# pityka/lamp

Hardware: AMD Instinct MI355X
Metric: training-step samples/sec (higher is better)
Workload: dtype bf16; 1 GPU; example-cifar100 Cnn.resnet(100) training step (fwd+backprop+AdamW), synthetic CIFAR batch; per_gpu_batch=2048, global_batch=2048, parallelism=single, optimizer=AdamW lr 1e-3 wd 0 beta2 0.95 mixedPrecision

## Files before the change

### lamp_amd/csrc/core/switches.h

```cpp
#pragma once
#include <cstdint>

namespace lamp {

constexpr int64_t SW_NO_CLAMP = INT64_MIN;

#define LAMP_SWITCHES_ONCE(X)                                                                                                             \
                                                        \
  X(conv_sibling, "LAMP_CONV_SIBLING", BOOL, 1, 0, "a residual block's 3x3 and its sibling 1x1 of the same input as one forward launch") \
  X(fuse_bn_pair, "LAMP_FUSE_BN_PAIR", BOOL, 1, 0, "relu(bn(right) + bn(left)) at a block's end as one op (0: the chain)")                \
  X(fuse_pool_logsoftmax, "LAMP_FUSE_POOL_LOGSOFTMAX", BOOL, 1, 0, "average pool -> flatten -> log-softmax tail as one node")             \
  X(fuse_block_tail, "LAMP_FUSE_BLOCK_TAIL", BOOL, 1, 0, "the last residual block and the pooled log-softmax tail as one node")          \
  X(fuse_bn_conv, "LAMP_FUSE_BN_CONV", BOOL, 1, 0, "batch norm -> relu -> convolution: the convolution applies the norm while staging")  \
  X(fuse_loss_accumulate, "LAMP_FUSE_LOSS_ACCUMULATE", BOOL, 1, 0, "acc += n * loss inside the NLL loss kernel")                          \
  X(fuse_loss_backward, "LAMP_FUSE_LOSS_BACKWARD", BOOL, 1, 0, "the NLL loss backward goes straight to the pooled log-softmax node's input in one launch")                      \
  X(fuse_loss_tail, "LAMP_FUSE_LOSS_TAIL", BOOL, 1, 0, "the loss launch also writes the pooled log-softmax's input gradient per plane")  \
  X(conv_dgrad_accumulate, "LAMP_CONV_DGRAD_ACCUMULATE", BOOL, 1, 0, "a convolution's input gradient adds into the existing one in its epilogue") \
  X(conv_dgrad_pair, "LAMP_CONV_DGRAD_PAIR", BOOL, 1, 0, "input gradients of a block's 3x3 and sibling 1x1 from one launch")             \
  X(conv_wgrad_pair, "LAMP_CONV_WGRAD_PAIR", BOOL, 1, 0, "weight gradients of a block's 3x3 and sibling 1x1 from one launch")            \
  X(linear_bias_fused, "LAMP_LINEAR_BIAS_FUSED", BOOL, 1, 0, "a linear layer's bias in the GEMM epilogue (0: mm then add)")               \
  X(mult_add_fused, "LAMP_MULT_ADD_FUSED", BOOL, 1, 0, "x * scale + residual in one pass (0: mult then add)")                             \
  X(attention_as_written_for_cuda, "LAMP_ATTENTION_AS_WRITTEN_FOR_CUDA", BOOL, 0, 0, "multi-head attention as the reference's op chain instead of the fused kernels") \
  X(recurrent_fused, "LAMP_RECURRENT_FUSED", BOOL, 1, 0, "RNN / GRU / LSTM as one node per sequence with fused cell kernels (0: the fold over time steps)") \
  X(fuse_qkv, "LAMP_FUSE_QKV", BOOL, 1, 0, "self-attention's three projections as one product (0: three)")                                \
  X(host_stream_side, "LAMP_HOST_STREAM_SIDE", BOOL, 0, 0, "batch streams gather on a side stream instead of the consumer's")             \
                                                                           \
  X(pinned_cache_mb, "LAMP_PINNED_CACHE_MB", INT, 2048, 0, "upper bound of the cache of freed pinned host buffers, MiB")                  \
  X(pinned_gather_wgs, "LAMP_PINNED_GATHER_WGS", INT, 48, 1, "workgroups of a gather that reads pinned host memory")                      \
                                                                                                    \
  X(flash_attention, "LAMP_FLASH_ATTENTION", BOOL, 1, 0, "the flash attention kernels, forward and backward")                             \
  X(small_attention, "LAMP_SMALL_ATTENTION", BOOL, 1, 0, "the short-sequence attention kernels")                                          \
  X(knn_fused, "LAMP_KNN_FUSED", BOOL, 1, 0, "the fused distance + top-k nearest-neighbour kernel")                                       \
  X(knn_split, "LAMP_KNN_SPLIT", INT, -1, SW_NO_CLAMP, "f16-plane k-NN filter: 0 off, 1 where it pays, 2 forced; negative: the mode set through the API") \
  X(knn_split_planes, "LAMP_KNN_SPLIT_PLANES", INT, 0, SW_NO_CLAMP, "f16 planes per coordinate of that filter: 3, anything else 2")      \
  X(umap_pairs2, "LAMP_UMAP_PAIRS2", BOOL, 1, 0, "the UMAP loss's two-dimensional pair kernel")                                            \
                                                                                                             \
  X(gemm_shape_tags, "LAMP_GEMM_SHAPE_TAGS", BOOL, 0, 0, "profiling aid: one kernel-timer class per GEMM shape and layout")               \
  X(gemm_splitk, "LAMP_GEMM_SPLITK", BOOL, 1, 0, "split-K for products with few output tiles (bf16 and f32 / f64)")                       \
  X(gemm_tail_split, "LAMP_GEMM_TAIL_SPLIT", BOOL, 1, 0, "an almost empty last round of 256 x 256 tiles becomes a second, split-K product") \
  X(gemm_fp_split_wgs, "LAMP_GEMM_FP_SPLIT_WGS", INT, 512, 1, "workgroups an f32 / f64 split-K product aims at")                          \
                                                                                              \
  X(bn_fused_bwd, "LAMP_BN_FUSED_BWD", BOOL, 1, 0, "one-pass batch-norm backward (workgroups exchange their sums) where no mode is set through the API") \
  X(bn_fused_fp, "LAMP_BN_FUSED_FP", BOOL, 1, 0, "... its f32 / f64 form")                                                               \
  X(bn_fused_np_mask, "LAMP_BN_FUSED_NP_MASK", INT, 24, SW_NO_CLAMP, "bit mask of packets per thread (1 .. 16) at which the one-pass form runs") \
  X(bn_fused_per_cu, "LAMP_BN_FUSED_PER_CU", INT, 1, 1, "workgroups per CU the one-pass form aims at first")                              \
  X(bn_fused_small_bytes, "LAMP_BN_FUSED_SMALL_BYTES", INT, (4 << 20) + 1, SW_NO_CLAMP, "bf16 activations below this many bytes take the one-pass form whatever the mask") \
                          \
  X(conv_small2, "LAMP_CONV_SMALL2", BOOL, 1, 0, "the small-map direct convolution kernels (second generation)")                          \
  X(conv_small2_wgrad, "LAMP_CONV_SMALL2_WGRAD", BOOL, 1, 0, "... their weight gradient")                                                 \
  X(igemm_f32, "LAMP_IGEMM_F32", BOOL, 1, 0, "implicit-GEMM convolution for f32")                                                          \
  X(igemm_f64, "LAMP_IGEMM_F64", BOOL, 1, 0, "implicit-GEMM convolution for f64")                                                          \
  X(conv_bn_stats, "LAMP_CONV_BN_STATS", BOOL, 1, 0, "forward convolutions hand per-image batch-norm statistics of their output on")     \
  X(ncv_bn_stats, "LAMP_NCV_BN_STATS", BOOL, 1, 0, "... the narrow kernels' alone (needs LAMP_CONV_BN_STATS on as well)")                 \
  X(ncv_dgrad_parity, "LAMP_NCV_DGRAD_PARITY", BOOL, 1, 0, "narrow stride-2 pair input gradient: super-tiles by row parity (0: the plain form)") \
  X(ncv_pitch, "LAMP_NCV_PITCH", BOOL, 1, 0, "narrow kernels widen the LDS row pitch to a bank-conflict-free one")                        \
  X(ncv_two_shift, "LAMP_NCV_TWO_SHIFT", BOOL, 1, 0, "narrow kernels: two output phases per MFMA where the columns allow it")             \
  X(ncv_per_cu, "LAMP_NCV_PER_CU", INT, 4, 1, "narrow kernels: most workgroups per CU")                                                   \
  X(pack_cache, "LAMP_PACK_CACHE", BOOL, 1, 0, "packed filter images are cached per parameter and storage version (all four packing backends: core/pack_cache.h)") \
  X(pack_after_step, "LAMP_PACK_AFTER_STEP", BOOL, 1, 0, "the optimiser repacks every cached filter image of all four backends in place (0: lazily at first use)") \
                                                    \
  X(ig_small_d, "LAMP_IG_SMALL_D", BOOL, 1, 0, "the eight-image kernel for at most 64 output channels too")                               \
  X(ig_w8, "LAMP_IG_W8", BOOL, 1, 0, "two-image 128-row kernel: eight waves per image pair at one workgroup per CU or fewer (0: four)")  \
  X(ig_one_image, "LAMP_IG_ONE_IMAGE", BOOL, 1, 0, "... one image per workgroup at one image per CU or fewer (0: pairs)")                 \
                                                                                                 \
  X(wgrad_group, "LAMP_WGRAD_GROUP", BOOL, 1, 0, "two layers' eight-wave weight gradients parked and launched as one (0: every layer at once)") \
  X(wgrad_min_ips, "LAMP_WGRAD_MIN_IPS", INT, 0, 2, "fewest images per weight-gradient workgroup; unset (0): 2 up to 512 images, 8 above") \
  X(wg8h_dma, "LAMP_WG8H_DMA", BOOL, 1, 0, "eight-wave weight-gradient kernel: dY tiles by LDS-DMA (0: through registers, the bitwise reference of the DMA's hand-counted waits)") \
  X(defer_wgrad_reduce, "LAMP_DEFER_WGRAD_REDUCE", BOOL, 1, 0, "weight-gradient partial sums are reduced in batches, deferred until someone reads them")

#define LAMP_SWITCHES_PER_CALL(X)                                                                                                         \
  X(ig_variant, "LAMP_IG_VARIANT", LETTER, 0, 0, "bf16 implicit GEMM kernel form: b two-image 128-row, d eight-image at any batch; unset or any other letter: by geometry") \
  X(ig_ktail, "LAMP_IG_KTAIL", BOOL, 1, 0, "a 3x3's 1 .. 8 channels beyond the last whole K chunk from their own packed image (0: the padded chunk)") \
  X(knn_split_dbg, "LAMP_KNN_SPLIT_DBG", INT, 0, SW_NO_CLAMP, "3: the k-NN filter's kernel counts visits, candidates and selection cycles per wave and prints them")

using SwType_BOOL = bool;
using SwType_INT = int64_t;
using SwType_LETTER = char;
#define LAMP_SWITCH_MEMBER(member, name, kind, dflt, lo, doc) SwType_##kind member;
struct Switches { LAMP_SWITCHES_ONCE(LAMP_SWITCH_MEMBER) };
struct SwitchesNow { LAMP_SWITCHES_PER_CALL(LAMP_SWITCH_MEMBER) };
#undef LAMP_SWITCH_MEMBER

const Switches& sw();
SwitchesNow sw_now();

}
```

### lamp_amd/csrc/kernels/conv_igemm.hip

```cpp
#include "device_utils.h"
#include "conv_geom.h"
#include "conv_backends.h"
#include "../core/pack_cache.h"
#include "wgrad_reduce.h"
#include <thread>
#include "conv_narrow_pack.h"
#include "../core/switches.h"

namespace lamp {

typedef short s8v __attribute__((ext_vector_type(8)));
typedef __bf16 bf8v __attribute__((ext_vector_type(8)));
typedef float f4v __attribute__((ext_vector_type(4)));

constexpr int IG_M = 128;
constexpr int IG_WTILE = 128 * 64 * 2;

__device__ __forceinline__ int ig_kc_off(int row, int chunk) { return row * 128 + ((chunk ^ (row & 7)) << 4); }

__device__ __forceinline__ void ig_stage_load_rows(uint4 (&r)[4], const bf16_t* __restrict__ base, int64_t ld, int64_t k0, int64_t rows,
                                                   int64_t K, int tid) {
#pragma unroll
  for (int i = 0; i < 4; i++) {
    const int c = tid + i * 256;
// ... 487 lines not shown
    const int qrow = (q == 1 || q == 2) ? 1 : 0, qw = (q >= 2) ? 4 : 0;
#pragma unroll
    for (int i = 0; i < 2; i++) {
      const int co = wr * 32 + i * 16 + (lane & 15);
      const float b = (bias && co < CO) ? (float)bias[co] : 0.f;
      float vals[16];
#pragma unroll
      for (int j = 0; j < 4; j++) {
        const bf16_t o0(acc[i][j][0] + b), o1(acc[i][j][1] + b), o2(acc[i][j][2] + b), o3(acc[i][j][3] + b);
        if (co < CO) {
          uint2 pk;
          pk.x = (unsigned)o0.bits | ((unsigned)o1.bits << 16);
          pk.y = (unsigned)o2.bits | ((unsigned)o3.bits << 16);
          if (addend) {
            const uint2 av = *reinterpret_cast<const uint2*>(addend + (int64_t)n * CO * 64 + co * 64 + (2 * j + qrow) * 8 + qw);
            pk.x = add_bf16x2(pk.x, av.x); pk.y = add_bf16x2(pk.y, av.y);
          }
          *reinterpret_cast<uint2*>(yp + co * 64 + (2 * j + qrow) * 8 + qw) = pk;
        }
        vals[4 * j + 0] = __uint_as_float((unsigned)o0.bits << 16); vals[4 * j + 1] = __uint_as_float((unsigned)o1.bits << 16);
        vals[4 * j + 2] = __uint_as_float((unsigned)o2.bits << 16); vals[4 * j + 3] = __uint_as_float((unsigned)o3.bits << 16);
      }
      if (stats) {
        float wn, wm, w2;
        ig_stats_wave(vals, wn, wm, w2);
        if (q == 0 && co < CO) { float* sp = stats + ((int64_t)co * N + n) * 3;  sp[0] = wn; sp[1] = wm; sp[2] = w2; }
      }
    }
  }
}

__device__ __forceinline__ uint4 ig_bn_relu_x8(uint4 v, float mu, float scale, float bb) {
  unsigned* w = &v.x;
#pragma unroll
  for (int q = 0; q < 4; q++) {
    const float x0 = __uint_as_float(w[q] << 16), x1 = __uint_as_float(w[q] & 0xffff0000u);
    bf16_t o0(__builtin_fmaf(x0 - mu, scale, bb)), o1(__builtin_fmaf(x1 - mu, scale, bb));
    if ((float)o0 < 0.f) o0 = bf16_t(0.f);
    if ((float)o1 < 0.f) o1 = bf16_t(0.f);
    w[q] = (unsigned)o0.bits | ((unsigned)o1.bits << 16);
  }
  return v;
}

#ifdef IG8D_STAMP
__device__ unsigned long long ig8d_stamps[8 * 512];
__device__ unsigned long long ig8d_rt_stamps[8 * 512];
#define IG_STAMP(k) do { if (threadIdx.x == 0 && blockIdx.x < 512) { ig8d_stamps[blockIdx.x * 8 + (k)] = __builtin_amdgcn_s_memtime(); \
                                                                     ig8d_rt_stamps[blockIdx.x * 8 + (k)] = __builtin_amdgcn_s_memrealtime(); } } while (0)
#else
#define IG_STAMP(k) do { } while (0)
#endif
__device__ __forceinline__ int ig8d_swz(int h, int w) { return ((h & 1) << 1) | ((w >> 2) & 1); }

__device__ __forceinline__ void ig8d_tile_stats(const uint2 (&pk)[4], float& mean, float& m2) {
  typedef float f2v __attribute__((ext_vector_type(2)));
  const float sh = __uint_as_float(pk[0].x << 16);
  const f2v sh2 = {sh, sh};
  f2v s1 = {0.f, 0.f}, s2 = {0.f, 0.f};
#pragma unroll
  for (int j = 0; j < 4; j++) {
    const f2v va = {__uint_as_float(pk[j].x << 16), __uint_as_float(pk[j].x & 0xffff0000u)};
    const f2v vb = {__uint_as_float(pk[j].y << 16), __uint_as_float(pk[j].y & 0xffff0000u)};
    const f2v da = va - sh2, db = vb - sh2;
    s1 += da; s2 = __builtin_elementwise_fma(da, da, s2);
    s1 += db; s2 = __builtin_elementwise_fma(db, db, s2);
  }
  const float t1 = s1[0] + s1[1], t2 = s2[0] + s2[1];
  mean = sh + t1 * (1.f / 16.f); m2 = t2 - t1 * t1 * (1.f / 16.f);
  {
    float ma = mean, mb = mean, qa = m2, qb = m2;
    asm("s_nop 1\n\tv_permlane16_swap_b32 %0, %1" : "+v"(ma), "+v"(mb));
    asm("s_nop 1\n\tv_permlane16_swap_b32 %0, %1" : "+v"(qa), "+v"(qb));
    const float d = mb - ma; mean = ma + d * 0.5f; m2 = qa + qb + d * d * 8.f;
  }
  {
    float ma = mean, mb = mean, qa = m2, qb = m2;
    asm("s_nop 1\n\tv_permlane32_swap_b32 %0, %1" : "+v"(ma), "+v"(mb));
    asm("s_nop 1\n\tv_permlane32_swap_b32 %0, %1" : "+v"(qa), "+v"(qb));
    const float d = mb - ma; mean = ma + d * 0.5f; m2 = qa + qb + d * d * 16.f;
  }
}

template <int KS, int NCT, int SIBM>
__global__ __launch_bounds__(512) void ig_conv8d_kernel(const bf16_t* __restrict__ x, const bf16_t* __restrict__ wp, const bf16_t* __restrict__ bias,
                                                        bf16_t* y, int N, int CI, int KP, int CO, float* __restrict__ stats, int stats_per_wg,
                                                        const bf16_t* addend, const float4* __restrict__ affine, const IgSibling sib) {
  constexpr bool SIB = SIBM == 1, DG2 = SIBM == 2;
  static_assert(SIBM == 0 || KS == 3, "the sibling product is the centre tap of a 3x3 staging");
  extern __shared__ __attribute__((aligned(16))) char smem[];
  constexpr int RS = KS * KS;
  constexpr int PAD = (KS - 1) / 2;
  constexpr int NI = 8, NT = 512;
  constexpr int WT = 128 * 32 * 2, NSLOT = 3;
  constexpr int RB = 64;
  constexpr int XIMG = 64 * RB;
  constexpr int XBUF = NI * XIMG;
  char* Wl = smem;
  char* Xl = smem + NSLOT * WT;
  const int tid = threadIdx.x, lane = tid & 63;
  const int wid = __builtin_amdgcn_readfirstlane(tid >> 6);
  const int grp = wid >> 2;
  const int n0 = blockIdx.x * NI;
  const int KC = (CI + 31) >> 5;
  const bool tailm = KS == 3 && !SIB && sib.wtail != nullptr;
  const int KCF = tailm ? KC - 1 : KC;
  const int T = RS * KCF + (tailm ? IG_TAIL_STAGES : 0);

  typedef __attribute__((address_space(3))) char lds_char_t;
  typedef const __attribute__((address_space(1))) char glb_char_t;
  const int d_row = wid * 16 + (lane >> 2);
  const unsigned d_src = (unsigned)(d_row * KP + (((lane & 3) ^ ((4 - ((d_row >> 2) & 3)) & 3)) << 3)) * 2u;
  const unsigned d_src4 = d_src + 64u * (unsigned)KP * 2u;
  constexpr int NPIECE = SIB ? 2 : 1;
  const bool dma_wave = SIB ? wid < 4 : wid < NCT;
  auto stage_dma_of = [&](const bf16_t* wimg, int kc1, int rs1, int slot) {
    const char* base = reinterpret_cast<const char*>(wimg + (int64_t)rs1 * IG_M * KP + kc1 * 32);
    if constexpr (SIB) {
      if (wid < 4) {
        __builtin_amdgcn_global_load_lds((glb_char_t*)(base + d_src), (lds_char_t*)(Wl + slot * WT + wid * 1024), 16, 0, 0);
        __builtin_amdgcn_global_load_lds((glb_char_t*)(base + d_src4), (lds_char_t*)(Wl + slot * WT + (wid + 4) * 1024), 16, 0, 0);
      }
    } else {
      if (wid < NCT)
        __builtin_amdgcn_global_load_lds((glb_char_t*)(base + d_src), (lds_char_t*)(Wl + slot * WT + wid * 1024), 16, 0, 0);
    }
  };
  const unsigned d_srct = (unsigned)(d_row * 32 + (((lane & 3) ^ ((4 - ((d_row >> 2) & 3)) & 3)) << 3)) * 2u;
  auto stage_dma = [&](int kc1, int rs1, int slot) {
    if (kc1 < KCF) { stage_dma_of(wp, kc1, rs1, slot); return; }
    if constexpr (!SIB) {
      const char* base = reinterpret_cast<const char*>(sib.wtail + ((kc1 - KCF) * RS + rs1) * (IG_M * 32));
      if (wid < NCT) __builtin_amdgcn_global_load_lds((glb_char_t*)(base + d_srct), (lds_char_t*)(Wl + slot * WT + wid * 1024), 16, 0, 0);
    }
  };
  constexpr bool WIDE = NCT == 1 && !SIB;
  const unsigned d_srcw = (unsigned)((lane >> 2) * KP + wid * 32 + (((lane & 3) ^ ((4 - ((lane >> 4) & 3)) & 3)) << 3)) * 2u;
  auto stage_dma_w = [&](const bf16_t* wimg, int rs1, int slot) {
    if (wid < KC)
      __builtin_amdgcn_global_load_lds((glb_char_t*)(reinterpret_cast<const char*>(wimg + (int64_t)rs1 * IG_M * KP) + d_srcw),
                                       (lds_char_t*)(Wl + slot * WT + wid * 1024), 16, 0, 0);
  };
  const bool taps4 = WIDE && !DG2 && KC == 1 && RS > 1;
  auto stage_dma_t = [&](int g, int slot) {
    const int tap = 4 * g + wid;
    if (wid < 4 && tap < RS)
      __builtin_amdgcn_global_load_lds((glb_char_t*)(reinterpret_cast<const char*>(wp + (int64_t)tap * IG_M * KP) + (d_srcw - (unsigned)(wid * 32) * 2u)),
                                       (lds_char_t*)(Wl + slot * WT + wid * 1024), 16, 0, 0);
  };
  IG_STAMP(0);
  if constexpr (WIDE) {
    if (taps4) { stage_dma_t(0, 0); stage_dma_t(1, 1); }
    else if (DG2) { stage_dma_w(sib.wp, 0, 0); stage_dma_w(wp, 0, 1); }
    else { stage_dma_w(wp, 0, 0); if (RS > 1) stage_dma_w(wp, 1, 1); }
  } else if (SIB || DG2) {
    stage_dma_of(sib.wp, 0, 0, 0);
    if (KC > 1) stage_dma_of(sib.wp, 1, 0, 1);
  } else {
    stage_dma(0, 0, 0);
    if (T > 1) stage_dma(1 / RS, 1 % RS, 1);
  }
  IG_STAMP(1);
  unsigned bpair[SIB ? (NCT + 1) / 2 : 1];
  if constexpr (SIB) {
#pragma unroll
    for (int k = 0; k < (NCT + 1) / 2; k++) {
      const int c0 = 2 * k * 16 + (lane & 15), c1 = c0 + 16;
      const unsigned b0 = (sib.bias && c0 < CO) ? sib.bias[c0].bits : 0u, b1 = (sib.bias && 2 * k + 1 < NCT && c1 < CO) ? sib.bias[c1].bits : 0u;
      bpair[k] = b0 | (b1 << 16);
    }
  }
  auto load_images = [&](const bf16_t* __restrict__ x) {
    for (int e = tid; e < NI * 8 * 4 * KC; e += NT) {
      const int cg = e & 3, h = (e >> 2) & 7, img = (e >> 5) & 7, ch = e >> 8;
      const int n = n0 + img;
      uint4 rw[8];
#pragma unroll
      for (int k = 0; k < 8; k++) {
        const int c = ch * 32 + cg * 8 + k;
        rw[k] = make_uint4(0, 0, 0, 0);
        if (c < CI && n < N) {
          const uint4* src = reinterpret_cast<const uint4*>(x + ((int64_t)n * CI + c) * 64 + h * 8);
          rw[k] = stats ? nt_load16(src) : *src;
        }
      }
      if (affine) {
#pragma unroll
        for (int k = 0; k < 8; k++) {
          const int c = ch * 32 + cg * 8 + k;
          if (c < CI && n < N) { const float4 a = affine[c]; rw[k] = ig_bn_relu_x8(rw[k], a.x, a.y, a.z); }
        }
      }
      char* xi = Xl + ch * XBUF + img * XIMG;
#pragma unroll
      for (int p = 0; p < 8; p++) {
        unsigned int d[4];
#pragma unroll
        for (int j = 0; j < 4; j++) {
          const unsigned int lo = (&rw[2 * j].x)[p >> 1], hi = (&rw[2 * j + 1].x)[p >> 1];
          d[j] = (p & 1) ? ((lo >> 16) | (hi & 0xffff0000u)) : ((lo & 0xffffu) | (hi << 16));
        }
        *reinterpret_cast<uint4*>(xi + (h * 8 + p) * RB + ((cg ^ ig8d_swz(h, p)) << 4)) = make_uint4(d[0], d[1], d[2], d[3]);
      }
    }
  };
  load_images(DG2 ? sib.x2 : x);
  f4v acc[NCT][4];
#pragma unroll
  for (int i = 0; i < NCT; i++)
#pragma unroll
    for (int j = 0; j < 4; j++) acc[i][j] = f4v{0.f, 0.f, 0.f, 0.f};

  int rowsel, wpix;
  px_of_col(lane & 15, rowsel, wpix);
  const int p0 = wid * XIMG + ((rowsel - PAD) * 8 + (wpix - PAD)) * RB;
  int va[2][KS];
#pragma unroll
  for (int par = 0; par < 2; par++)
#pragma unroll
    for (int s = 0; s < KS; s++)
      va[par][s] = p0 + (((lane >> 4) ^ ig8d_swz(rowsel + par - PAD, wpix + s - PAD)) << 4);
  const bool col_lo = wpix == 0, col_hi = wpix == 7, row_lo = rowsel == 0, row_hi = rowsel == 1;
  const int a_off = (lane & 15) * 64 + ((((lane >> 4) ^ ((4 - ((lane >> 2) & 3)) & 3)) & 3) << 4);

  asm volatile("s_waitcnt vmcnt(0) lgkmcnt(0)" ::: "memory");
  __builtin_amdgcn_s_barrier();
  if constexpr (SIB) {
#pragma unroll
    for (int k = 0; k < (NCT + 1) / 2; k++) asm volatile("" : "+v"(bpair[k]));
  }
  IG_STAMP(2);

  bf8v fa[NCT], fb[4];
  const bf8v zero8 = __builtin_bit_cast(bf8v, s8v{0, 0, 0, 0, 0, 0, 0, 0});
  if constexpr (WIDE) {
    bf8v fw[4], fx[4][4];
    auto read_stage = [&](int slot, int r, int s) {
      const char* wl = Wl + slot * WT + a_off;
#pragma unroll
      for (int kc = 0; kc < 4; kc++)
        if (kc < KC) {
          fw[kc] = __builtin_bit_cast(bf8v, *reinterpret_cast<const s8v*>(wl + kc * 1024));
          const char* xb = Xl + kc * XBUF + va[r & 1][s];
#pragma unroll
          for (int j = 0; j < 4; j++) fx[kc][j] = __builtin_bit_cast(bf8v, *reinterpret_cast<const s8v*>(xb + ((r * 8 + s) + 16 * j) * RB));
        }
    };
    auto zero_outside = [&](int r, int s) {
      if (KS != 3) return;
      const bool colout = (s == 0 && col_lo) || (s == 2 && col_hi);
#pragma unroll
      for (int kc = 0; kc < 4; kc++)
        if (kc < KC) {
#pragma unroll
          for (int j = 0; j < 4; j++) {
            const bool out = colout || (r == 0 && j == 0 && row_lo) || (r == 2 && j == 3 && row_hi);
            if (s != 1 || (r == 0 && j == 0) || (r == 2 && j == 3)) fx[kc][j] = out ? zero8 : fx[kc][j];
          }
        }
    };
    auto multiply = [&] {
      __builtin_amdgcn_s_setprio(1);
#pragma unroll
      for (int kc = 0; kc < 4; kc++)
        if (kc < KC) {
#pragma unroll
          for (int j = 0; j < 4; j++) acc[0][j] = __builtin_amdgcn_mfma_f32_16x16x32_bf16(fx[kc][j], fw[kc], acc[0][j], 0, 0, 0);
        }
      __builtin_amdgcn_s_setprio(0);
    };
    int slot = 0;
    if (taps4) {
      constexpr int NG = (RS + 3) / 4;
      if (grp == 1) __builtin_amdgcn_s_barrier();
#pragma unroll
      for (int g = 0; g < NG; g++) {
        const int slot1 = slot == 2 ? 0 : slot + 1, slot2 = slot1 == 2 ? 0 : slot1 + 1;
        if (g + 2 < NG) stage_dma_t(g + 2, slot2);
        const char* wl = Wl + slot * WT + a_off;
#pragma unroll
        for (int p = 0; p < 4; p++) {
          const int tap = 4 * g + p;
          if (tap < RS) {
            const int r = tap / KS, s_ = tap - r * KS;
            fw[p] = __builtin_bit_cast(bf8v, *reinterpret_cast<const s8v*>(wl + p * 1024));
            const char* xb = Xl + va[r & 1][s_];
#pragma unroll
            for (int j = 0; j < 4; j++) fx[p][j] = __builtin_bit_cast(bf8v, *reinterpret_cast<const s8v*>(xb + ((r * 8 + s_) + 16 * j) * RB));
          }
        }
        if (g + 2 < NG) asm volatile("s_waitcnt vmcnt(1) lgkmcnt(0)" ::: "memory");
        else asm volatile("s_waitcnt vmcnt(0) lgkmcnt(0)" ::: "memory");
        if (KS == 3) {
#pragma unroll
          for (int p = 0; p < 4; p++) {
            const int tap = 4 * g + p;
            if (tap < RS) {
              const int r = tap / KS, s_ = tap - r * KS;
              const bool colout = (s_ == 0 && col_lo) || (s_ == 2 && col_hi);
#pragma unroll
              for (int j = 0; j < 4; j++) {
                const bool out = colout || (r == 0 && j == 0 && row_lo) || (r == 2 && j == 3 && row_hi);
                if (s_ != 1 || (r == 0 && j == 0) || (r == 2 && j == 3)) fx[p][j] = out ? zero8 : fx[p][j];
              }
            }
          }
        }
        __builtin_amdgcn_s_barrier();
        __builtin_amdgcn_s_setprio(1);
#pragma unroll
        for (int p = 0; p < 4; p++)
          if (4 * g + p < RS) {
// ... 741 lines not shown
      if (co < CO2 && ci < CI) __builtin_nontemporal_store(acc2[i], reinterpret_cast<f4v*>(&out2[co * CIP + ci]));
    }
  }
#pragma unroll
  for (int t = 0; t < RS; t++) {
    float* out = partial + (int64_t)(split * RS + t) * IG_M * CIP;
#pragma unroll
    for (int i = 0; i < 2; i++) {
      const int ci = ci0 + i * 16 + (lane >> 4) * 4;
      if (co < CO && ci < CI) __builtin_nontemporal_store(acc[t][i], reinterpret_cast<f4v*>(&out[co * CIP + ci]));
    }
  }
}

static bool ig_qualifies(const ConvGeom& g, int dtype) {
  if (dtype != kBF16) return false;
  if (g.groups != 1 || g.transposed) return false;
  if (g.H != 8 || g.W != 8 || g.Ho != 8 || g.Wo != 8) return false;
  if (g.sh != 1 || g.sw != 1 || g.dh != 1 || g.dw != 1) return false;
  if (!((g.kh == 3 && g.kw == 3 && g.ph == 1 && g.pw == 1) || (g.kh == 1 && g.kw == 1 && g.ph == 0 && g.pw == 0))) return false;
  if (g.Cin > 128 || g.Cout > 128 || g.Cin < 8 || g.Cout < 8) return false;
  if (g.N < 1) return false;
  return true;
}
static int pad_k(int64_t c) { return c <= 64 ? 64 : 128; }

static PackCache g_ig_packs;

static Tensor* packed_weights(const Tensor* w, const ConvGeom& g, int KS, hipStream_t st, int64_t* dgrad_offset, int64_t* tail_offset = nullptr) {
  const int RS = KS * KS;
  const int KPf = pad_k(g.Cin), KPd = pad_k(g.Cout);
  const int64_t nf = (int64_t)RS * IG_M * KPf, nd = (int64_t)RS * IG_M * KPd;
  const int64_t ntf = ig_tail_ok((int)g.Cin, KS) ? IG_TAIL_ELEMS : 0, ntd = ig_tail_ok((int)g.Cout, KS) ? IG_TAIL_ELEMS : 0;
  *dgrad_offset = nf;
  if (tail_offset) { tail_offset[0] = ntf ? nf + nd : -1; tail_offset[1] = ntd ? nf + nd + ntf : -1; }
  const bool cacheable = PackCache::cacheable(w);
  const PackKey key = PackKey::filter(w, KS, (int)g.Cout, (int)g.Cin, st);
  const uint64_t ver = PackCache::version_of(w);
  if (cacheable) if (Tensor* hit = g_ig_packs.find(key, ver)) return hit;
  int64_t ps[1] = {nf + nd + ntf + ntd};
  Hold wp(new_tensor(ps, 1, kBF16, w->device()));
  hipLaunchKernelGGL(ig_pack_weights_kernel, dim3(grid_for(ps[0], 256)), dim3(256), 0, st, w->ptr<bf16_t>(), wp->ptr<bf16_t>(), (int)g.Cout,
                     (int)g.Cin, KS, KPf, KPd);
  LAMP_LAUNCH_CHECK();
  if (cacheable) g_ig_packs.insert(key, ver, 0, wp.get());
  return wp.take();
}

void igemm_repack_cached(lamp_tensor* const* params, int n, hipStream_t st) {
  NcvPackMany nb;
  int ncnt = 0;
  narrow_repack_cached(params, n, st, &nb, &ncnt);
  PackMany a;
  int maxtotal = 0;
  static_assert(NCV_NKMAX * 64 <= 4 * 256, "a narrow image is four blocks of the pack kernel");
  g_ig_packs.repack(params, n, st, kBF16, IG_PACK_MAX,
      [&](int slot, const Tensor* w, const PackKey& k, Tensor* packed) {
        const int KS = k.tag[0], Cout = k.tag[1], Cin = k.tag[2];
        const int total = KS * KS * IG_M * (pad_k(Cin) + pad_k(Cout)) + (ig_tail_ok(Cin, KS) ? IG_TAIL_ELEMS : 0) + (ig_tail_ok(Cout, KS) ? IG_TAIL_ELEMS : 0);
        if (packed->numel() != total) return false;
        a.w[slot] = w->ptr<bf16_t>(); a.Cout[slot] = Cout; a.Cin[slot] = Cin; a.KS[slot] = KS; a.KPf[slot] = pad_k(Cin); a.KPd[slot] = pad_k(Cout);
        a.wp[slot] = static_cast<bf16_t*>(packed->raw());
        maxtotal = std::max(maxtotal, total);
        return true;
      },
      [&](int cnt, bool last) {
        const unsigned gx = (unsigned)std::min(512, (maxtotal + 255) / 256);
        if (last && ncnt > 0 && 4 * ncnt <= (int)gx) {
          hipLaunchKernelGGL(ig_ncv_pack_many_kernel, dim3(gx, (unsigned)(cnt + 1)), dim3(256), 0, st, a, nb, cnt, ncnt);
          ncnt = 0;
        } else {
          hipLaunchKernelGGL(ig_pack_weights_many_kernel, dim3(gx, (unsigned)cnt), dim3(256), 0, st, a);
        }
        LAMP_LAUNCH_CHECK();
        maxtotal = 0;
      });
  if (ncnt > 0) narrow_pack_launch(nb, ncnt, st);
}

enum class IgForm { Eight, Two64, Two128 };
static IgForm ig_form(const ConvGeom& g, bool dgrad) {
  const char variant = sw_now().ig_variant;
  const int64_t CO = dgrad ? g.Cin : g.Cout;
  if ((CO > 64 || sw().ig_small_d) && variant != 'b' && (variant == 'd' || g.N >= 4 * (int64_t)num_cus())) return IgForm::Eight;
  return (CO <= 64 && variant != 'b') ? IgForm::Two64 : IgForm::Two128;
}

struct SiblingConv { const Tensor* w; const Tensor* bias; Tensor* out; const ConvGeom* g; };
struct SecondGradConv { const Tensor* dy; const Tensor* w; const ConvGeom* g; };
struct IgRequest {
  const Tensor* addend = nullptr;
  const Tensor* affine = nullptr;
  const SiblingConv* sibling = nullptr;
  const SecondGradConv* second = nullptr;
};
struct IgPlan {
  IgForm form;
  bool folds_addend, folds_affine;
  bool sibling, second;
  bool stats, per_wg;
  bool w8, one;
  int blocks;
  size_t lds;
};
static IgPlan ig_plan(const ConvGeom& g, bool dgrad, const IgRequest& rq) {
  IgPlan p{};
  p.form = ig_form(g, dgrad);
  const int KS = g.kh, CI = (int)(dgrad ? g.Cout : g.Cin), KP = pad_k(CI);
  const bool eight = p.form == IgForm::Eight;
  auto beside = [&](const ConvGeom* o) { return KS == 3 && o->kh == 1 && o->Cout == g.Cout && o->Cin == g.Cin && o->N == g.N; };
  p.folds_addend = eight || dgrad;
  p.folds_affine = eight;
  p.sibling = sw().conv_sibling && rq.sibling && !dgrad && !rq.addend && p.form != IgForm::Two64 && beside(rq.sibling->g);
  p.second = sw().conv_dgrad_pair && rq.second && dgrad && beside(rq.second->g);
  p.stats = sw().conv_bn_stats && !dgrad && g.N >= 2;
  const int pairs = (int)((g.N + 1) / 2);
  if (eight) {
    p.blocks = (int)((g.N + 7) / 8);
    p.per_wg = p.stats && g.N % 8 == 0;
    p.lds = std::max<size_t>((size_t)3 * (128 * 32 * 2) + (size_t)((CI + 31) / 32) * 8 * 4096 + (KS == 3 ? 9 * 64 : 0), (size_t)8 * 16384 + 8 * 128 * 8);
  } else if (p.form == IgForm::Two64) {
    p.blocks = pairs;
    p.lds = (size_t)2 * 64 * KP * 2 + KP * 2 + 4 * (64 * 64 * 2);
  } else {
    p.w8 = sw().ig_w8 && pairs <= num_cus();
    p.one = sw().ig_one_image && p.w8 && g.N <= num_cus();
    p.blocks = p.one ? (int)g.N : pairs;
    p.lds = (size_t)(p.one ? 1 : 2) * 64 * KP * 2 + KP * 2 + (p.one ? 4 : 2) * IG_WTILE;
  }
  return p;
}

struct StatsPublish { Hold& t; const Tensor* y; int P; ~StatsPublish() { if (t.get()) conv_stats_publish(y, t.get(), P); } };

static IgSibling ig_second_product(const IgRequest& rq, const IgPlan& pl, int64_t stat_elems, hipStream_t st, Hold* wpk, Hold* statt) {
  IgSibling s{nullptr, nullptr, nullptr, nullptr, nullptr, nullptr};
  if (!pl.sibling && !pl.second) return s;
  int64_t dgrad_off = 0;
  *wpk = Hold(pl.second ? packed_weights(rq.second->w, *rq.second->g, 1, st, &dgrad_off) : packed_weights(rq.sibling->w, *rq.sibling->g, 1, st, &dgrad_off));
  s.wp = static_cast<const Tensor*>(wpk->get())->ptr<bf16_t>() + (pl.second ? dgrad_off : 0);
  if (pl.second) { s.x2 = rq.second->dy->ptr<bf16_t>(); return s; }
  s.bias = rq.sibling->bias ? rq.sibling->bias->ptr<bf16_t>() : (const bf16_t*)nullptr;
  s.y = rq.sibling->out->ptr<bf16_t>();
  if (stat_elems) {
    int64_t ps[1] = {stat_elems};
    *statt = Hold(new_tensor(ps, 1, kF32, rq.sibling->out->device()));
    s.stats = (*statt)->ptr<float>();
  }
  return s;
}

static void run_conv8(const Tensor* in, const Tensor* w, const Tensor* bias, Tensor* out, const ConvGeom& g, bool dgrad, hipStream_t st,
                      const IgRequest& rq, const IgPlan& pl) {
  const int KS = g.kh;
  const int CI = (int)(dgrad ? g.Cout : g.Cin), CO = (int)(dgrad ? g.Cin : g.Cout);
  const int KP = pad_k(CI);
  int64_t dgrad_off = 0;
  int64_t tail_off[2] = {-1, -1};
  Hold wpk(packed_weights(w, g, KS, st, &dgrad_off, tail_off));
  const bf16_t* wpp = static_cast<const Tensor*>(wpk.get())->ptr<bf16_t>() + (dgrad ? dgrad_off : 0);
  const bool ktail_on = sw_now().ig_ktail;
  const bf16_t* wtailp = (ktail_on && tail_off[dgrad ? 1 : 0] >= 0) ? static_cast<const Tensor*>(wpk.get())->ptr<bf16_t>() + tail_off[dgrad ? 1 : 0] : (const bf16_t*)nullptr;
  const int64_t stat_elems = pl.stats ? (int64_t)g.N * CO * 3 : 0;
  Hold statt;
  float* statp = nullptr;
  if (stat_elems) {
    int64_t ps[1] = {stat_elems};
    statt = Hold(new_tensor(ps, 1, kF32, in->device()));
    statp = statt->ptr<float>();
  }
  const int per_wg = pl.per_wg ? 1 : 0;
  StatsPublish publish{statt, out, per_wg ? pl.blocks : (int)g.N};
  const ConvGeom* g2 = pl.sibling ? rq.sibling->g : pl.second ? rq.second->g : nullptr;
  const double fl2 = g2 ? conv_flops(*g2) : 0.0, by2 = g2 ? conv_bytes(*g2, 2) - (double)g.N * g.Cin * 64 * 2 : 0.0;
  KernelTimer kt("conv_igemm_fprop_dgrad", conv_flops(g) + fl2, conv_bytes(g, 2) + by2, st);
  const bf16_t* bp = bias ? bias->ptr<bf16_t>() : (const bf16_t*)nullptr;
  const bf16_t* addp = (rq.addend && pl.folds_addend) ? rq.addend->ptr<bf16_t>() : (const bf16_t*)nullptr;
  const float4* affp = (rq.affine && pl.folds_affine) ? reinterpret_cast<const float4*>(rq.affine->ptr<float>()) : (const float4*)nullptr;
  Hold sib_wpk, sib_statt;
  StatsPublish publish_sib{sib_statt, pl.sibling ? rq.sibling->out : nullptr, publish.P};
  IgSibling sib = ig_second_product(rq, pl, stat_elems, st, &sib_wpk, &sib_statt);
  const int sibm = pl.second ? 2 : pl.sibling ? 1 : 0;
  const int N = (int)g.N;
  const bf16_t* inp = in->ptr<bf16_t>();
  bf16_t* outp = out->ptr<bf16_t>();
#define IG_FOR_KS_SIBM(L_)                                                                                                                     \
  do { if (KS == 1) L_(1, 0); else if (sibm == 2) L_(3, 2); else if (sibm == 1) L_(3, 1); else L_(3, 0); } while (0)
  if (pl.form == IgForm::Eight) {
    if (KS == 3 && CO > 16 && !pl.sibling) sib.wtail = wtailp;
#define IG_LAUNCH_D(KS_, NCT_, SIBM_)                                                                                                          \
  do {                                                                                                                                         \
    allow_big_lds((const void*)ig_conv8d_kernel<KS_, NCT_, SIBM_>);                                                                            \
    hipLaunchKernelGGL((ig_conv8d_kernel<KS_, NCT_, SIBM_>), dim3(pl.blocks), dim3(512), pl.lds, st, inp, wpp, bp, outp, N, CI, KP, CO, statp, \
                       per_wg, addp, affp, sib);                                                                                               \
  } while (0)
#define IG_LAUNCH_D_CO(KS_, SIBM_)                                                                                                             \
  do { if (CO <= 16) IG_LAUNCH_D(KS_, 1, SIBM_); else if (CO <= 64) IG_LAUNCH_D(KS_, 4, SIBM_); else if (CO <= 112) IG_LAUNCH_D(KS_, 7, SIBM_); \
       else IG_LAUNCH_D(KS_, 8, SIBM_); } while (0)
    IG_FOR_KS_SIBM(IG_LAUNCH_D_CO);
#undef IG_LAUNCH_D_CO
#undef IG_LAUNCH_D
  } else {
#define IG_LAUNCH_TWO(K_, NT_)                                                                                                                 \
  do {                                                                                                                                         \
    allow_big_lds((const void*)K_);                                                                                                            \
    hipLaunchKernelGGL(K_, dim3(pl.blocks), dim3(NT_), pl.lds, st, inp, wpp, bp, outp, N, CI, KP, CO, statp, addp, sib);                       \
  } while (0)
#define IG_LAUNCH_B(KS_, SIBM_)                                                                                                                \
  do { if (pl.one) IG_LAUNCH_TWO((ig_conv8b_kernel<KS_, 8, SIBM_, 1>), 512); else if (pl.w8) IG_LAUNCH_TWO((ig_conv8b_kernel<KS_, 8, SIBM_, 2>), 512); \
       else IG_LAUNCH_TWO((ig_conv8b_kernel<KS_, 4, SIBM_, 2>), 256); } while (0)
    if (pl.form == IgForm::Two128) IG_FOR_KS_SIBM(IG_LAUNCH_B);
    else if (KS == 1) IG_LAUNCH_TWO((ig_conv8c_kernel<1>), 256);
    else if (sibm == 2) IG_LAUNCH_TWO((ig_conv8c_kernel<3, 2>), 256);
    else IG_LAUNCH_TWO((ig_conv8c_kernel<3>), 256);
#undef IG_LAUNCH_B
#undef IG_LAUNCH_TWO
  }
#undef IG_FOR_KS_SIBM
  LAMP_LAUNCH_CHECK();
}

bool igemm_conv_fwd(const Tensor* x, const Tensor* w, const Tensor* bias, Tensor* y, const ConvGeom& g, hipStream_t st) {
  if (!ig_qualifies(g, x->dtype)) return false;
  const IgRequest rq;
  run_conv8(x, w, bias, y, g, false, st, rq, ig_plan(g, false, rq));
  return true;
}
bool igemm_conv_fwd_pair(const Tensor* x, const Tensor* w, const Tensor* bias, Tensor* y, const ConvGeom& g, const Tensor* w1, const Tensor* bias1,
                         Tensor* y1, const ConvGeom& g1, hipStream_t st) {
  if (!ig_qualifies(g, x->dtype) || !ig_qualifies(g1, x->dtype)) return false;
  const SiblingConv sc{w1, bias1, y1, &g1};
  IgRequest rq;
  rq.sibling = &sc;
  const IgPlan pl = ig_plan(g, false, rq);
  if (!pl.sibling) return false;
  run_conv8(x, w, bias, y, g, false, st, rq, pl);
  return true;
}
bool igemm_conv_dgrad_pair(const Tensor* dy, const Tensor* w, const ConvGeom& g, const Tensor* dy1, const Tensor* w1, const ConvGeom& g1, Tensor* dx,
                           hipStream_t st, const Tensor* addend, bool* addend_fused) {
  if (addend_fused) *addend_fused = false;
  if (!ig_qualifies(g, dy->dtype) || !ig_qualifies(g1, dy1->dtype)) return false;
  const SecondGradConv sg{dy1, w1, &g1};
  IgRequest rq;
  rq.addend = addend;
  rq.second = &sg;
  const IgPlan pl = ig_plan(g, true, rq);
  if (!pl.second) return false;
  run_conv8(dy, w, nullptr, dx, g, true, st, rq, pl);
  if (addend_fused) *addend_fused = addend && pl.folds_addend;
  return true;
}
static bool ig_fwd_folds_affine(const ConvGeom& g, int dtype) { return ig_qualifies(g, dtype) && ig_plan(g, false, IgRequest{}).folds_affine; }
static bool wgrad_takes_eight_wave(const ConvGeom& g) { return g.kh == 3 && g.Cin > WG_CI && g.Cout > 64; }
static bool ig_wgrad_folds_affine(const ConvGeom& g, int dtype) { return ig_qualifies(g, dtype) && wgrad_takes_eight_wave(g); }
bool igemm_conv_folds_affine(const ConvGeom& g, int dtype) { return ig_fwd_folds_affine(g, dtype) && ig_wgrad_folds_affine(g, dtype); }
bool igemm_conv_fwd_affine(const Tensor* x, const Tensor* affine, const Tensor* w, const Tensor* bias, Tensor* y, const ConvGeom& g, hipStream_t st) {
  if (!ig_qualifies(g, x->dtype)) return false;
  IgRequest rq;
  rq.affine = affine;
  const IgPlan pl = ig_plan(g, false, rq);
  if (!pl.folds_affine) return false;
  run_conv8(x, w, bias, y, g, false, st, rq, pl);
  return true;
}
bool igemm_conv_dgrad(const Tensor* dy, const Tensor* w, Tensor* dx, const ConvGeom& g, hipStream_t st, const Tensor* addend, bool* addend_fused) {
  if (addend_fused) *addend_fused = false;
  if (!ig_qualifies(g, dy->dtype)) return false;
  IgRequest rq;
  rq.addend = addend;
  const IgPlan pl = ig_plan(g, true, rq);
  run_conv8(dy, w, nullptr, dx, g, true, st, rq, pl);
  if (addend_fused) *addend_fused = addend && pl.folds_addend;
  return true;
}
static int wgrad_min_ips(int64_t N) {
  const int v = (int)sw().wgrad_min_ips;
  return v ? v : (N <= 512 ? 2 : 8);
}
struct WgradSplit { int ips, nsplit; };
static WgradSplit wgrad_split(int64_t N, int wg_budget, int ntile) {
  const int target = std::max(1, wg_budget / ntile);
// ... 154 lines not shown
```

Baseline: 2.209 million samples/s.

## Add sliced eight-image forward 3x3 conv form for narrow-input layers

Adds a sliced variant of the eight-image implicit-GEMM forward kernel for 3x3 convolutions with at most 32 input channels and more than 64 outputs. The variant loads all nine tap weight tiles (plus the sibling 1x1) into LDS at once, keeps the input fragments in registers, and walks output channel tiles in pairs. Each pair gets its own epilogue for bias, bf16 pack, stats and store, which avoids the per-tap weight streaming of the serial form. It uses more LDS and registers, which may reduce occupancy. By default it applies whenever the geometry qualifies.

```diff
diff --git a/lamp_amd/csrc/core/switches.h b/lamp_amd/csrc/core/switches.h
--- a/lamp_amd/csrc/core/switches.h
+++ b/lamp_amd/csrc/core/switches.h
@@ -69,7 +69,7 @@
   X(defer_wgrad_reduce, "LAMP_DEFER_WGRAD_REDUCE", BOOL, 1, 0, "weight-gradient partial sums are reduced in batches, deferred until someone reads them")
 
 #define LAMP_SWITCHES_PER_CALL(X)                                                                                                         \
-  X(ig_variant, "LAMP_IG_VARIANT", LETTER, 0, 0, "bf16 implicit GEMM kernel form: b two-image 128-row, d eight-image at any batch; unset or any other letter: by geometry") \
+  X(ig_variant, "LAMP_IG_VARIANT", LETTER, 0, 0, "bf16 implicit GEMM kernel form: b two-image 128-row, d eight-image at any batch in its serial form, s eight-image at any batch and sliced where the geometry allows; unset or any other letter: by geometry") \
   X(ig_ktail, "LAMP_IG_KTAIL", BOOL, 1, 0, "a 3x3's 1 .. 8 channels beyond the last whole K chunk from their own packed image (0: the padded chunk)") \
   X(knn_split_dbg, "LAMP_KNN_SPLIT_DBG", INT, 0, SW_NO_CLAMP, "3: the k-NN filter's kernel counts visits, candidates and selection cycles per wave and prints them")
 
diff --git a/lamp_amd/csrc/kernels/conv_igemm.hip b/lamp_amd/csrc/kernels/conv_igemm.hip
--- a/lamp_amd/csrc/kernels/conv_igemm.hip
+++ b/lamp_amd/csrc/kernels/conv_igemm.hip
@@ -593,17 +593,18 @@
   }
 }
 
-template <int KS, int NCT, int SIBM>
+template <int KS, int NCT, int SIBM, bool SLICED = false>
 __global__ __launch_bounds__(512) void ig_conv8d_kernel(const bf16_t* __restrict__ x, const bf16_t* __restrict__ wp, const bf16_t* __restrict__ bias,
                                                         bf16_t* y, int N, int CI, int KP, int CO, float* __restrict__ stats, int stats_per_wg,
                                                         const bf16_t* addend, const float4* __restrict__ affine, const IgSibling sib) {
   constexpr bool SIB = SIBM == 1, DG2 = SIBM == 2;
   static_assert(SIBM == 0 || KS == 3, "the sibling product is the centre tap of a 3x3 staging");
+  static_assert(!SLICED || (KS == 3 && NCT == 8 && SIBM != 2), "the sliced form: forward 3x3, four slices of two channel tiles");
   extern __shared__ __attribute__((aligned(16))) char smem[];
   constexpr int RS = KS * KS;
   constexpr int PAD = (KS - 1) / 2;
   constexpr int NI = 8, NT = 512;
-  constexpr int WT = 128 * 32 * 2, NSLOT = 3;
+  constexpr int WT = 128 * 32 * 2, NSLOT = SLICED ? 1 + RS : 3;
   constexpr int RB = 64;
   constexpr int XIMG = 64 * RB;
   constexpr int XBUF = NI * XIMG;
@@ -660,7 +661,13 @@
                                        (lds_char_t*)(Wl + slot * WT + wid * 1024), 16, 0, 0);
   };
   IG_STAMP(0);
-  if constexpr (WIDE) {
+  if constexpr (SLICED) {
+#pragma unroll
+    for (int g = SIB ? 0 : 1; g < NSLOT; g++) {
+      const char* base = reinterpret_cast<const char*>(g == 0 ? sib.wp : wp + (int64_t)(g - 1) * IG_M * KP);
+      __builtin_amdgcn_global_load_lds((glb_char_t*)(base + d_src), (lds_char_t*)(Wl + g * WT + wid * 1024), 16, 0, 0);
+    }
+  } else if constexpr (WIDE) {
     if (taps4) { stage_dma_t(0, 0); stage_dma_t(1, 1); }
     else if (DG2) { stage_dma_w(sib.wp, 0, 0); stage_dma_w(wp, 0, 1); }
     else { stage_dma_w(wp, 0, 0); if (RS > 1) stage_dma_w(wp, 1, 1); }
@@ -673,12 +680,26 @@
   }
   IG_STAMP(1);
   unsigned bpair[SIB ? (NCT + 1) / 2 : 1];
-  if constexpr (SIB) {
+  if constexpr (SIB && !SLICED) {
 #pragma unroll
     for (int k = 0; k < (NCT + 1) / 2; k++) {
       const int c0 = 2 * k * 16 + (lane & 15), c1 = c0 + 16;
       const unsigned b0 = (sib.bias && c0 < CO) ? sib.bias[c0].bits : 0u, b1 = (sib.bias && 2 * k + 1 < NCT && c1 < CO) ? sib.bias[c1].bits : 0u;
       bpair[k] = b0 | (b1 << 16);
+    }
+  }
+  unsigned bown[SLICED ? NCT / 2 : 1];
+  if constexpr (SLICED) {
+    auto pair_of = [&](const bf16_t* bsrc, int k) {
+      const int c0 = 2 * k * 16 + (lane & 15), c1 = c0 + 16;
+      const bf16_t* src = bsrc ? bsrc : wp;
+      const unsigned v0 = src[min(c0, CO - 1)].bits, v1 = src[min(c1, CO - 1)].bits;
+      return ((bsrc && c0 < CO) ? v0 : 0u) | (((bsrc && c1 < CO) ? v1 : 0u) << 16);
+    };
+#pragma unroll
+    for (int k = 0; k < NCT / 2; k++) {
+      bown[k] = pair_of(bias, k);
+      if constexpr (SIB) bpair[k] = pair_of(sib.bias, k);
     }
   }
   auto load_images = [&](const bf16_t* __restrict__ x) {
@@ -739,6 +760,130 @@
   if constexpr (SIB) {
 #pragma unroll
     for (int k = 0; k < (NCT + 1) / 2; k++) asm volatile("" : "+v"(bpair[k]));
+  }
+  if constexpr (SLICED) {
+#pragma unroll
+    for (int k = 0; k < NCT / 2; k++) asm volatile("" : "+v"(bown[k]));
+    IG_STAMP(2);
+    typedef float f2v __attribute__((ext_vector_type(2)));
+    typedef __bf16 bf2v __attribute__((ext_vector_type(2)));
+    const bf8v zero8 = __builtin_bit_cast(bf8v, s8v{0, 0, 0, 0, 0, 0, 0, 0});
+    const int q = lane >> 4, cl = lane & 15;
+    const int qrow = (q == 1 || q == 2) ? 1 : 0, qw = (q >= 2) ? 4 : 0;
+    bf8v fx[RS][4];
+#pragma unroll
+    for (int rs = 0; rs < RS; rs++) {
+      const int r = rs / KS, s = rs - r * KS;
+      const char* xb = Xl + va[r & 1][s];
+#pragma unroll
+      for (int j = 0; j < 4; j++) fx[rs][j] = __builtin_bit_cast(bf8v, *reinterpret_cast<const s8v*>(xb + ((r * 8 + s) + 16 * j) * RB));
+    }
+#pragma unroll
+    for (int rs = 0; rs < RS; rs++) {
+      const int r = rs / KS, s = rs - r * KS;
+      const bool colout = (s == 0 && col_lo) || (s == 2 && col_hi);
+#pragma unroll
+      for (int j = 0; j < 4; j++) {
+        const bool out = colout || (r == 0 && j == 0 && row_lo) || (r == 2 && j == 3 && row_hi);
+        if (s != 1 || (r == 0 && j == 0) || (r == 2 && j == 3)) {
+          s8v f = __builtin_bit_cast(s8v, fx[rs][j]);
+          asm volatile("" : "+v"(f));
+          fx[rs][j] = out ? zero8 : __builtin_bit_cast(bf8v, f);
+        }
+      }
+    }
+    char* El = Xl + XBUF + 1024 + wid * 4096;
+    float2* St = reinterpret_cast<float2*>(Xl + wid * XIMG);
+    const int64_t yoff = (int64_t)(n0 + wid) * CO * 64;
+    auto leave = [&](const f4v (&a)[2][4], int p, unsigned bp, bf16_t* dst, float2* st) {
+#pragma unroll
+      for (int t = 0; t < 2; t++) {
+        const int cr = t * 16 + cl;
+        const float b = __uint_as_float(t ? (bp & 0xffff0000u) : (bp << 16));
+        uint2 pk[4];
+#pragma unroll
+        for (int j = 0; j < 4; j++) {
+          const f2v lo = {a[t][j][0] + b, a[t][j][1] + b}, hi = {a[t][j][2] + b, a[t][j][3] + b};
+          pk[j].x = __builtin_bit_cast(unsigned, __builtin_convertvector(lo, bf2v));
+          pk[j].y = __builtin_bit_cast(unsigned, __builtin_convertvector(hi, bf2v));
+          const int sl = (2 * j + qrow) * 2 + (qw >> 2);
+          *reinterpret_cast<uint2*>(El + cr * 128 + ((sl ^ ((cr & 7) << 1)) << 3)) = pk[j];
+        }
+        if (st) {
+          float mean, m2;
+          ig8d_tile_stats(pk, mean, m2);
+          if (q == 0) st[p * 32 + cr] = make_float2(mean, m2);
+        }
+      }
+      s8v v[4];
+#pragma unroll
+      for (int it = 0; it < 4; it++) {
+        const int idx = it * 64 + lane;
+        const int cr = idx >> 3, c = idx & 7;
+        v[it] = *reinterpret_cast<const s8v*>(El + cr * 128 + ((c ^ (cr & 7)) << 4));
+      }
+      asm volatile("" : "+v"(v[0]), "+v"(v[1]), "+v"(v[2]), "+v"(v[3]));
+#pragma unroll
+      for (int it = 0; it < 4; it++) {
+        const int idx = it * 64 + lane;
+        const int cr = idx >> 3, c = idx & 7, co = p * 32 + cr;
+        if (co < CO) {
+          const uint4 u = __builtin_bit_cast(uint4, v[it]);
+          *reinterpret_cast<uint4*>(dst + co * 64 + c * 8) = u;
+        }
+      }
+    };
+    auto multiply = [&](f4v (&a)[2][4], int g, int p, const bf8v (&f)[4]) {
+      const char* wl = Wl + g * WT + 2 * p * 1024 + a_off;
+      const bf8v w0 = __builtin_bit_cast(bf8v, *reinterpret_cast<const s8v*>(wl));
+      const bf8v w1 = __builtin_bit_cast(bf8v, *reinterpret_cast<const s8v*>(wl + 1024));
+#pragma unroll
+      for (int j = 0; j < 4; j++) a[0][j] = __builtin_amdgcn_mfma_f32_16x16x32_bf16(f[j], w0, a[0][j], 0, 0, 0);
+#pragma unroll
+      for (int j = 0; j < 4; j++) a[1][j] = __builtin_amdgcn_mfma_f32_16x16x32_bf16(f[j], w1, a[1][j], 0, 0, 0);
+    };
+#pragma unroll
+    for (int p = 0; p < NCT / 2; p++) {
+      if (p * 32 < CO) {
+        f4v a[2][4];
+        if constexpr (SIB) {
+#pragma unroll
+          for (int t = 0; t < 2; t++)
+#pragma unroll
+            for (int j = 0; j < 4; j++) a[t][j] = f4v{0.f, 0.f, 0.f, 0.f};
+          multiply(a, 0, p, fx[PAD * KS + PAD]);
+          leave(a, p, bpair[p], sib.y + yoff, sib.stats ? St + 128 : nullptr);
+        }
+#pragma unroll
+        for (int t = 0; t < 2; t++)
+#pragma unroll
+          for (int j = 0; j < 4; j++) a[t][j] = f4v{0.f, 0.f, 0.f, 0.f};
+#pragma unroll
+        for (int rs = 0; rs < RS; rs++) multiply(a, 1 + rs, p, fx[rs]);
+        leave(a, p, bown[p], y + yoff, stats ? St : nullptr);
+      }
+    }
+    IG_STAMP(3); IG_STAMP(4); IG_STAMP(5);
+    if (stats || (SIB && sib.stats)) {
+      asm volatile("s_waitcnt lgkmcnt(0)" ::: "memory");
+      __builtin_amdgcn_s_barrier();
+      const int prod = tid >> 8, ch = tid & 255;
+      float* table = prod ? (SIB ? sib.stats : nullptr) : stats;
+      if (table && ch < CO) {
+        const float2* sl = reinterpret_cast<const float2*>(Xl) + prod * 128 + ch;
+        const float shift = sl[0].x;
+        float s1 = 0.f, s2 = 0.f, sm = 0.f;
+#pragma unroll
+        for (int w = 0; w < 8; w++) { const float2 v = sl[w * (XIMG / 8)]; const float d = v.x - shift; s1 += d; s2 += d * d; sm += v.y; }
+        float* sp = table + ((int64_t)ch * gridDim.x + blockIdx.x) * 3;
+        sp[0] = 512.f; sp[1] = shift + s1 * 0.125f; sp[2] = sm + 64.f * (s2 - s1 * s1 * 0.125f);
+      }
+    }
+#ifdef IG8D_STAMP
+    asm volatile("s_waitcnt vmcnt(0)" ::: "memory");
+    IG_STAMP(6);
+#endif
+    return;
   }
   IG_STAMP(2);
 
@@ -1646,7 +1791,7 @@
 static IgForm ig_form(const ConvGeom& g, bool dgrad) {
   const char variant = sw_now().ig_variant;
   const int64_t CO = dgrad ? g.Cin : g.Cout;
-  if ((CO > 64 || sw().ig_small_d) && variant != 'b' && (variant == 'd' || g.N >= 4 * (int64_t)num_cus())) return IgForm::Eight;
+  if ((CO > 64 || sw().ig_small_d) && variant != 'b' && (variant == 'd' || variant == 's' || g.N >= 4 * (int64_t)num_cus())) return IgForm::Eight;
   return (CO <= 64 && variant != 'b') ? IgForm::Two64 : IgForm::Two128;
 }
 
@@ -1664,6 +1809,7 @@
   bool sibling, second;
   bool stats, per_wg;
   bool w8, one;
+  bool sliced;
   int blocks;
   size_t lds;
 };
@@ -1682,7 +1828,9 @@
   if (eight) {
     p.blocks = (int)((g.N + 7) / 8);
     p.per_wg = p.stats && g.N % 8 == 0;
+    p.sliced = !dgrad && KS == 3 && CI <= 32 && g.Cout > 64 && g.N % 8 == 0 && !rq.addend && sw_now().ig_variant != 'd';
     p.lds = std::max<size_t>((size_t)3 * (128 * 32 * 2) + (size_t)((CI + 31) / 32) * 8 * 4096 + (KS == 3 ? 9 * 64 : 0), (size_t)8 * 16384 + 8 * 128 * 8);
+    if (p.sliced) p.lds = (size_t)10 * (128 * 32 * 2) + 8 * 4096 + 1024 + 8 * 4096;
   } else if (p.form == IgForm::Two64) {
     p.blocks = pairs;
     p.lds = (size_t)2 * 64 * KP * 2 + KP * 2 + 4 * (64 * 64 * 2);
@@ -1752,16 +1900,18 @@
   do { if (KS == 1) L_(1, 0); else if (sibm == 2) L_(3, 2); else if (sibm == 1) L_(3, 1); else L_(3, 0); } while (0)
   if (pl.form == IgForm::Eight) {
     if (KS == 3 && CO > 16 && !pl.sibling) sib.wtail = wtailp;
-#define IG_LAUNCH_D(KS_, NCT_, SIBM_)                                                                                                          \
+#define IG_LAUNCH_D(KS_, NCT_, ...)                                                                                                            \
   do {                                                                                                                                         \
-    allow_big_lds((const void*)ig_conv8d_kernel<KS_, NCT_, SIBM_>);                                                                            \
-    hipLaunchKernelGGL((ig_conv8d_kernel<KS_, NCT_, SIBM_>), dim3(pl.blocks), dim3(512), pl.lds, st, inp, wpp, bp, outp, N, CI, KP, CO, statp, \
-                       per_wg, addp, affp, sib);                                                                                               \
+    allow_big_lds((const void*)ig_conv8d_kernel<KS_, NCT_, __VA_ARGS__>);                                                                      \
+    hipLaunchKernelGGL((ig_conv8d_kernel<KS_, NCT_, __VA_ARGS__>), dim3(pl.blocks), dim3(512), pl.lds, st, inp, wpp, bp, outp, N, CI, KP, CO,  \
+                       statp, per_wg, addp, affp, sib);                                                                                        \
   } while (0)
 #define IG_LAUNCH_D_CO(KS_, SIBM_)                                                                                                             \
   do { if (CO <= 16) IG_LAUNCH_D(KS_, 1, SIBM_); else if (CO <= 64) IG_LAUNCH_D(KS_, 4, SIBM_); else if (CO <= 112) IG_LAUNCH_D(KS_, 7, SIBM_); \
        else IG_LAUNCH_D(KS_, 8, SIBM_); } while (0)
-    IG_FOR_KS_SIBM(IG_LAUNCH_D_CO);
+    LAMP_CHECK(!pl.sliced || !pl.stats || pl.per_wg, "conv_igemm: the sliced form needs whole workgroups of eight images");
+    if (pl.sliced) { if (sibm == 1) IG_LAUNCH_D(3, 8, 1, true); else IG_LAUNCH_D(3, 8, 0, true); }
+    else IG_FOR_KS_SIBM(IG_LAUNCH_D_CO);
 #undef IG_LAUNCH_D_CO
 #undef IG_LAUNCH_D
   } else {
```

Measured after the change: 2.235 million samples/s (median of 6 runs). 1.1% higher.
